# youtalk/opencv-ar

Hardware: AMD Instinct MI355X
Metric: frames/sec at 1920x1080, 16 markers/frame; 1/2/4/8 MI355X (higher is better)
Workload: dtype u8

## Files before the change

include/ocvar_hip.h:

```cpp
#ifndef OCVAR_HIP_H
#define OCVAR_HIP_H

#include <stddef.h>
#include <stdint.h>

#ifdef __cplusplus
extern "C" {
#endif

typedef struct { int width, height; double cameraMatrix[9]; double distCoeffs[5]; double glProjection[16]; } OcvarCamera;
typedef struct { int width, height; double scale; long long code[4]; } OcvarTemplate;
typedef struct {
    double glMatrix[16]; int templateId; int markerId; double score; float square[8]; double aspectRatio;
} OcvarMarker;

typedef struct {
    int markerId, templateId, orient, valid;
    long long bit;
    float square[8];
    float patPoint[8];
} OcvarCandidate;

typedef struct OcvarHip OcvarHip;

enum {
    OCVAR_OK = 0,
    OCVAR_E_NO_DEVICE = -1,
    OCVAR_E_ARG = -2,
    OCVAR_E_HIP = -3,
    OCVAR_E_CAPACITY = -4
};

enum { OCVAR_MAX_TEMPLATES = 4096, OCVAR_MAX_TEMPLATE_SIZES = 16, OCVAR_MAX_QUADS = 256, OCVAR_MAX_MARKERS = 64,
       OCVAR_MAX_QUADS_EX = 1792 ,
       OCVAR_MAX_QUADS_DENSE = 16384, OCVAR_MAX_MARKERS_DENSE = 4096  };

int ocvar_hip_create(OcvarHip** ctx, int device, int max_width, int max_height, int max_batch);
int ocvar_hip_create_ex(OcvarHip** ctx, int device, int max_width, int max_height, int max_batch, int max_quads);
int ocvar_hip_create_dense(OcvarHip** ctx, int device, int max_width, int max_height, int max_batch, int max_quads, int max_markers);
int ocvar_hip_max_markers(const OcvarHip* ctx);
void ocvar_hip_destroy(OcvarHip* ctx);
const char* ocvar_hip_last_error(const OcvarHip* ctx);
int ocvar_hip_capacity_flags(const OcvarHip* ctx);

typedef struct OcvarGate OcvarGate;
int ocvar_hip_gate_create(OcvarGate** gate, int device, int width);
int ocvar_hip_gate_create_lanes(OcvarGate** gate, int device, int width, int lanes);
int ocvar_hip_gate_lanes(const OcvarGate* gate);
void ocvar_hip_gate_destroy(OcvarGate* gate);
int ocvar_hip_set_gate(OcvarHip* ctx, OcvarGate* gate);

int ocvar_hip_set_templates(OcvarHip* ctx, const OcvarTemplate* templates, int n);
int ocvar_hip_set_camera(OcvarHip* ctx, const OcvarCamera* camera);

enum { OCVAR_FMT_BGR = 0, OCVAR_FMT_RGB = 1, OCVAR_FMT_BGRA = 2, OCVAR_FMT_RGBA = 3, OCVAR_FMT_GRAY = 4 };
int ocvar_hip_set_input_format(OcvarHip* ctx, int format);

enum { OCVAR_MAX_REFINE_HALF_WIN = 15 };
int ocvar_hip_set_corner_refine(OcvarHip* ctx, int half_win, int max_iter, float eps);

enum { OCVAR_MAX_BOARD_MARKERS = 256 };
typedef struct { int templateId; int pad; double corner[8]; } OcvarBoardMarker;
typedef struct {
    double glMatrix[16];
    double rvec[3], tvec[3];
    double rms;
    int n_markers;
    int status;
} OcvarBoardPose;
int ocvar_hip_set_board(OcvarHip* ctx, const OcvarBoardMarker* markers, int n);
int ocvar_hip_board_poses(OcvarHip* ctx, OcvarBoardPose* poses, int n_frames);
int ocvar_hip_board_poses_to_device(OcvarHip* ctx, OcvarBoardPose* d_poses, void* stream);

enum { OCVAR_MAX_OVERLAYS = 64, OCVAR_MAX_OVERLAY_SIDE = 1024 };
int ocvar_hip_set_overlay(OcvarHip* ctx, int template_id, const uint8_t* h_rgba, int width, int height, int row_stride);
int ocvar_hip_render(OcvarHip* ctx, uint8_t* d_frames, int width, int height, int row_stride, size_t frame_stride, int format,
                     void* stream);
int ocvar_hip_render_records(OcvarHip* ctx, uint8_t* d_frames, int width, int height, int row_stride, size_t frame_stride,
                             int n_frames, int format, const OcvarMarker* d_markers, const int* d_counts, int records_per_frame,
                             void* stream);

enum { OCVAR_MAX_PATCH_SIDE = 256, OCVAR_PATCH_FLIP_ROWS = 1, OCVAR_PATCH_MATCHED_ONLY = 2 };
int ocvar_hip_patches(OcvarHip* ctx, const uint8_t* d_frames, int width, int height, int row_stride, size_t frame_stride, int format,
                      uint8_t* d_patches, int patch_w, int patch_h, int records_per_frame, int flags, int* d_status, void* stream);
int ocvar_hip_patches_records(OcvarHip* ctx, const uint8_t* d_frames, int width, int height, int row_stride, size_t frame_stride,
                              int n_frames, int format, const OcvarMarker* d_markers, const int* d_counts, int records_per_frame,
                              uint8_t* d_patches, int patch_w, int patch_h, int flags, int* d_status, void* stream);

int ocvar_hip_detect_device(OcvarHip* ctx, uint8_t* d_bgr, int width, int height, int row_stride, size_t frame_stride,
                            int n_frames, int grey_in_place, const OcvarMarker* prev, const int* prev_counts,
                            OcvarMarker* markers, int* counts, int max_per_frame);
int ocvar_hip_enqueue(OcvarHip* ctx, uint8_t* d_bgr, int width, int height, int row_stride, size_t frame_stride,
                      int n_frames, int grey_in_place, const OcvarMarker* prev, const int* prev_counts, void* stream);
int ocvar_hip_collect(OcvarHip* ctx, OcvarMarker* markers, int* counts, int max_per_frame);
int ocvar_hip_enqueue_tracked(OcvarHip* ctx, uint8_t* d_bgr, int width, int height, int row_stride, size_t frame_stride,
                              int n_frames, int grey_in_place, const OcvarMarker* d_prev, const int* d_prev_counts, void* stream);
int ocvar_hip_ready(OcvarHip* ctx);
int ocvar_hip_set_result_limit(OcvarHip* ctx, int max_per_frame);

enum { OCVAR_TUNE_CROP_PHASES = 1,
       OCVAR_TUNE_MID_STEPS = 2,
       OCVAR_TUNE_MID_BLOCKS = 3, OCVAR_TUNE_LONG_BLOCKS = 4, OCVAR_TUNE_SHORT_BLOCKS = 5,
       OCVAR_TUNE_MIN_UNITS = 6,
       OCVAR_TUNE_GATE_MODE = 8,
       OCVAR_TUNE_HP_MASK = 7 };
int ocvar_hip_set_tuning(OcvarHip* ctx, int knob, int value);
const char* ocvar_hip_build_info(void);

void* ocvar_hip_stream(const OcvarHip* ctx);

int ocvar_hip_results_to_device(OcvarHip* ctx, OcvarMarker* d_markers, int* d_counts, void* stream);
int ocvar_hip_results_to_device_ex(OcvarHip* ctx, OcvarMarker* d_markers, int* d_counts, int max_per_frame, void* stream);

typedef struct OcvarPipe OcvarPipe;
int ocvar_hip_pipe_create(OcvarPipe** pipe, int device, int max_width, int max_height, int chunk_frames, int n_contexts, int gate_width);
void ocvar_hip_pipe_destroy(OcvarPipe* pipe);
const char* ocvar_hip_pipe_last_error(const OcvarPipe* pipe);
int ocvar_hip_pipe_set_templates(OcvarPipe* pipe, const OcvarTemplate* templates, int n);
int ocvar_hip_pipe_set_camera(OcvarPipe* pipe, const OcvarCamera* camera);
int ocvar_hip_pipe_detect_device(OcvarPipe* pipe, uint8_t* d_bgr, int width, int height, int row_stride, size_t frame_stride,
                                 long long n_frames, int grey_in_place, OcvarMarker* markers, int* counts, int max_per_frame);
int ocvar_hip_pipe_track_device(OcvarPipe* pipe, uint8_t* d_bgr, int width, int height, int row_stride, size_t frame_stride,
                                long long n_streams, int grey_in_place, int reset, OcvarMarker* markers, int* counts, int max_per_frame);

enum { OCVAR_E_BUSY = -6 };
int ocvar_hip_pipe_submit(OcvarPipe* pipe, uint8_t* d_bgr, int width, int height, int row_stride, size_t frame_stride, int n_frames,
                          int grey_in_place, long long tag);
int ocvar_hip_pipe_collect(OcvarPipe* pipe, long long* tag, OcvarMarker* markers, int* counts, int max_per_frame);
int ocvar_hip_pipe_in_flight(const OcvarPipe* pipe);
int ocvar_hip_pipe_set_result_limit(OcvarPipe* pipe, int max_per_frame);
int ocvar_hip_pipe_set_input_format(OcvarPipe* pipe, int format);
// ... 26 lines not shown
```

opencv-ar_amd/__init__.py:

```python
import ctypes as C
import os

import numpy as np

_HERE = os.path.dirname(os.path.abspath(__file__))
LIB_DIR = os.path.join(_HERE, "lib")
HIP_LIB = os.environ.get("OCVAR_HIP_LIB") or os.path.join(LIB_DIR, "libocvar_hip.so")
SYNTH_LIB = os.path.join(LIB_DIR, "libocvar_synth.so")
HOST_LIB = os.path.join(LIB_DIR, "libopencv-ar.so.1.0.0")

MAX_TEMPLATES, MAX_TEMPLATE_SIZES, MAX_QUADS, MAX_MARKERS = 4096, 16, 256, 64
MAX_QUADS_EX, MAX_QUADS_DENSE, MAX_MARKERS_DENSE = 1792, 16384, 4096

HIP_SYMBOLS = [
    "ocvar_hip_create", "ocvar_hip_create_ex", "ocvar_hip_create_dense", "ocvar_hip_max_markers", "ocvar_hip_capacity_flags", "ocvar_hip_gate_create", "ocvar_hip_gate_create_lanes", "ocvar_hip_gate_lanes", "ocvar_hip_gate_destroy", "ocvar_hip_set_gate", "ocvar_hip_ready", "ocvar_hip_set_result_limit",
    "ocvar_hip_pipe_create", "ocvar_hip_pipe_destroy", "ocvar_hip_pipe_last_error", "ocvar_hip_pipe_set_templates", "ocvar_hip_pipe_set_camera",
    "ocvar_hip_pipe_detect_device", "ocvar_hip_pipe_track_device", "ocvar_hip_pipe_submit", "ocvar_hip_pipe_collect", "ocvar_hip_pipe_in_flight", "ocvar_hip_pipe_set_result_limit", "ocvar_hip_set_input_format", "ocvar_hip_pipe_set_input_format", "ocvar_hip_set_corner_refine", "ocvar_hip_pipe_set_corner_refine", "ocvar_hip_enqueue_tracked", "ocvar_hip_build_info", "ocvar_hip_set_tuning", "ocvar_hip_destroy", "ocvar_hip_last_error", "ocvar_hip_set_templates", "ocvar_hip_set_camera",
    "ocvar_hip_detect_device", "ocvar_hip_enqueue", "ocvar_hip_collect", "ocvar_hip_detect_host", "ocvar_hip_find_squares",
    "ocvar_hip_debug_gray", "ocvar_hip_debug_binary", "ocvar_hip_debug_masks", "ocvar_hip_debug_frame_quads", "ocvar_hip_debug_candidates",
    "ocvar_hip_stage_ms", "ocvar_hip_stream", "ocvar_hip_stage_stamps", "ocvar_hip_counters", "ocvar_hip_results_to_device", "ocvar_hip_results_to_device_ex", "ocvar_hip_debug_calibrate",
    "ocvar_hip_set_board", "ocvar_hip_board_poses", "ocvar_hip_board_poses_to_device",
    "ocvar_hip_set_overlay", "ocvar_hip_render", "ocvar_hip_render_records",
    "ocvar_hip_patches", "ocvar_hip_patches_records",
]
INPUT_FORMATS = {"bgr": 0, "rgb": 1, "bgra": 2, "rgba": 3, "gray": 4}
FORMAT_BPP = {0: 3, 1: 3, 2: 4, 3: 4, 4: 1}


def input_format_code(fmt):
    if isinstance(fmt, str) and fmt.lower() in INPUT_FORMATS:
        return INPUT_FORMATS[fmt.lower()]
    if isinstance(fmt, int) and not isinstance(fmt, bool) and fmt in FORMAT_BPP:
        return fmt
    raise ValueError(f"unknown input format {fmt!r}: one of {sorted(INPUT_FORMATS)}")


def frame_shape_bpp(shape, fmt):
    bpp = FORMAT_BPP[input_format_code(fmt)]
    if bpp == 1:
        if len(shape) != 3:
            raise ValueError(f"gray frames are [n, H, W], got {tuple(shape)}")
    elif len(shape) != 4 or shape[3] != bpp:
        raise ValueError(f"frames in this format are [n, H, W, {bpp}], got {tuple(shape)}")
    return shape[0], shape[1], shape[2]


MAX_REFINE_HALF_WIN = 15


def corner_refine_args(half_win, max_iter, eps):
    for name, v in (("half_win", half_win), ("max_iter", max_iter)):
        if isinstance(v, bool) or not isinstance(v, (int, np.integer)):
            raise ValueError(f"{name} must be an int, got {v!r}")
    if not 0 <= half_win <= MAX_REFINE_HALF_WIN:
        raise ValueError(f"half_win must be 0 .. {MAX_REFINE_HALF_WIN}, got {half_win}")
    if not 1 <= max_iter <= 100:
        raise ValueError(f"max_iter must be 1 .. 100, got {max_iter}")
    if isinstance(eps, bool) or not isinstance(eps, (int, float, np.integer, np.floating)) or not 0 <= float(eps) < 1e30:
        raise ValueError(f"eps must be a number >= 0, got {eps!r}")
    return int(half_win), int(max_iter), float(eps)


MAX_BOARD_MARKERS = 256
MAX_OVERLAYS, MAX_OVERLAY_SIDE = 64, 1024
MAX_PATCH_SIDE, PATCH_FLIP_ROWS, PATCH_MATCHED_ONLY = 256, 1, 2


class BoardMarker(C.Structure):
    _fields_ = [("templateId", C.c_int), ("pad", C.c_int), ("corner", C.c_double * 8)]


BOARD_DTYPE = np.dtype([("glMatrix", "<f8", (16,)), ("rvec", "<f8", (3,)), ("tvec", "<f8", (3,)), ("rms", "<f8"),
                        ("n_markers", "<i4"), ("status", "<i4")], align=True)
assert C.sizeof(BoardMarker) == 72 and BOARD_DTYPE.itemsize == 192


def grid_board(template_ids, cols, rows, length, separation):
    if len(template_ids) > cols * rows:
        raise ValueError(f"{len(template_ids)} templates for a {cols} x {rows} grid")
    out = []
    for k, t in enumerate(template_ids):
        x0, y0 = (k % cols) * (length + separation), (k // cols) * (length + separation)
        out.append((int(t), np.array([[x0, y0], [x0 + length, y0], [x0 + length, y0 + length], [x0, y0 + length]], np.float64)))
    return out


STAGE_NAMES = ["binarise_frames", "follow1_frames", "follow2_frames", "follow3_frames", "order_crops", "binarise_crops",
               "follow1_crops", "follow2_crops", "follow3_crops", "decode", "dedupe_pose", "batch_total"]


class Camera(C.Structure):
    _fields_ = [("width", C.c_int), ("height", C.c_int), ("cameraMatrix", C.c_double * 9),
                ("distCoeffs", C.c_double * 5), ("glProjection", C.c_double * 16)]


class Template(C.Structure):
    _fields_ = [("width", C.c_int), ("height", C.c_int), ("scale", C.c_double), ("code", C.c_longlong * 4)]


class Marker(C.Structure):
    _fields_ = [("glMatrix", C.c_double * 16), ("templateId", C.c_int), ("markerId", C.c_int),
                ("score", C.c_double), ("square", C.c_float * 8), ("aspectRatio", C.c_double)]


class Candidate(C.Structure):
    _fields_ = [("markerId", C.c_int), ("templateId", C.c_int), ("orient", C.c_int), ("valid", C.c_int),
                ("bit", C.c_longlong), ("square", C.c_float * 8), ("patPoint", C.c_float * 8)]


MARKER_DTYPE = np.dtype([("glMatrix", "<f8", (16,)), ("templateId", "<i4"), ("markerId", "<i4"), ("score", "<f8"),
                         ("square", "<f4", (8,)), ("aspectRatio", "<f8")], align=True)
assert C.sizeof(Camera) == 248 and C.sizeof(Template) == 48 and C.sizeof(Marker) == 184 and MARKER_DTYPE.itemsize == 184


class OcvarError(RuntimeError):
    pass


_hip = None


def hip_lib():
    global _hip
    if _hip is None:
        if not os.path.exists(HIP_LIB):
            raise OcvarError(f"{HIP_LIB} is missing: run `python -c 'import __graft_entry__ as g; g.build()'` "
                             "(there is no CPU fallback for the detection path)")
        try:
            import torch
        except ImportError:
            pass
        lib = C.CDLL(HIP_LIB)
        vp, i, sz = C.c_void_p, C.c_int, C.c_size_t
        lib.ocvar_hip_create.argtypes = [C.POINTER(vp), i, i, i, i]
        lib.ocvar_hip_create_dense.argtypes = [C.POINTER(vp), i, i, i, i, i, i]
        lib.ocvar_hip_max_markers.argtypes = [vp]
        lib.ocvar_hip_destroy.argtypes = [vp]
        lib.ocvar_hip_gate_create.argtypes = [C.POINTER(vp), i, i]
        lib.ocvar_hip_gate_create_lanes.argtypes = [C.POINTER(vp), i, i, i]
        lib.ocvar_hip_gate_lanes.argtypes = [vp]
        lib.ocvar_hip_gate_destroy.argtypes = [vp]
        lib.ocvar_hip_gate_destroy.restype = None
        lib.ocvar_hip_set_gate.argtypes = [vp, vp]
        lib.ocvar_hip_ready.argtypes = [vp]
        lib.ocvar_hip_set_result_limit.argtypes = [vp, i]
        lib.ocvar_hip_pipe_create.argtypes = [C.POINTER(vp), i, i, i, i, i, i]
        lib.ocvar_hip_pipe_destroy.argtypes = [vp]
        lib.ocvar_hip_pipe_destroy.restype = None
        lib.ocvar_hip_pipe_last_error.argtypes = [vp]
        lib.ocvar_hip_pipe_last_error.restype = C.c_char_p
        lib.ocvar_hip_pipe_set_templates.argtypes = [vp, vp, i]
        lib.ocvar_hip_pipe_set_camera.argtypes = [vp, vp]
        lib.ocvar_hip_pipe_detect_device.argtypes = [vp, vp, i, i, i, sz, C.c_longlong, i, vp, vp, i]
        lib.ocvar_hip_pipe_track_device.argtypes = [vp, vp, i, i, i, sz, C.c_longlong, i, i, vp, vp, i]
        lib.ocvar_hip_pipe_submit.argtypes = [vp, vp, i, i, i, sz, i, i, C.c_longlong]
        lib.ocvar_hip_pipe_collect.argtypes = [vp, C.POINTER(C.c_longlong), vp, vp, i]
        lib.ocvar_hip_pipe_in_flight.argtypes = [vp]
        lib.ocvar_hip_pipe_set_result_limit.argtypes = [vp, i]
        lib.ocvar_hip_pipe_set_input_format.argtypes = [vp, i]
        lib.ocvar_hip_set_input_format.argtypes = [vp, i]
        lib.ocvar_hip_set_corner_refine.argtypes = [vp, i, i, C.c_float]
        lib.ocvar_hip_pipe_set_corner_refine.argtypes = [vp, i, i, C.c_float]
        lib.ocvar_hip_enqueue_tracked.argtypes = [vp, vp, i, i, i, sz, i, i, vp, vp, vp]
        lib.ocvar_hip_set_tuning.argtypes = [vp, i, i]
        lib.ocvar_hip_build_info.argtypes = []
        lib.ocvar_hip_build_info.restype = C.c_char_p
        lib.ocvar_hip_destroy.restype = None
        lib.ocvar_hip_last_error.argtypes = [vp]
        lib.ocvar_hip_last_error.restype = C.c_char_p
        lib.ocvar_hip_set_templates.argtypes = [vp, vp, i]
        lib.ocvar_hip_set_camera.argtypes = [vp, vp]
        lib.ocvar_hip_detect_device.argtypes = [vp, vp, i, i, i, sz, i, i, vp, vp, vp, vp, i]
        lib.ocvar_hip_enqueue.argtypes = [vp, vp, i, i, i, sz, i, i, vp, vp, vp]
        lib.ocvar_hip_collect.argtypes = [vp, vp, vp, i]
        lib.ocvar_hip_detect_host.argtypes = [vp, vp, i, i, i, sz, i, i, vp, vp, vp, vp, i]
        lib.ocvar_hip_find_squares.argtypes = [vp, vp, i, i, i, vp, i, vp]
        lib.ocvar_hip_debug_gray.argtypes = [vp, i, vp]
        lib.ocvar_hip_debug_binary.argtypes = [vp, i, vp]
        lib.ocvar_hip_debug_masks.argtypes = [vp, i, vp]
        lib.ocvar_hip_debug_frame_quads.argtypes = [vp, i, vp, vp]
        lib.ocvar_hip_debug_candidates.argtypes = [vp, i, vp, i, vp]
        lib.ocvar_hip_stage_ms.argtypes = [vp, vp, i]
        lib.ocvar_hip_counters.argtypes = [vp, vp, i]
        lib.ocvar_hip_stage_stamps.argtypes = [vp, vp, vp, i]
        lib.ocvar_hip_stream.argtypes = [vp]
        lib.ocvar_hip_stream.restype = vp
        lib.ocvar_hip_results_to_device.argtypes = [vp, vp, vp, vp]
        lib.ocvar_hip_results_to_device_ex.argtypes = [vp, vp, vp, i, vp]
        lib.ocvar_hip_debug_calibrate.argtypes = [vp, sz]
        lib.ocvar_hip_set_board.argtypes = [vp, vp, i]
        lib.ocvar_hip_board_poses.argtypes = [vp, vp, i]
        lib.ocvar_hip_board_poses_to_device.argtypes = [vp, vp, vp]
        lib.ocvar_hip_set_overlay.argtypes = [vp, i, vp, i, i, i]
        lib.ocvar_hip_render.argtypes = [vp, vp, i, i, i, sz, i, vp]
        lib.ocvar_hip_render_records.argtypes = [vp, vp, i, i, i, sz, i, i, vp, vp, i, vp]
        lib.ocvar_hip_patches.argtypes = [vp, vp, i, i, i, sz, i, vp, i, i, i, i, vp, vp]
        lib.ocvar_hip_patches_records.argtypes = [vp, vp, i, i, i, sz, i, i, vp, vp, i, vp, i, i, i, vp, vp]
        _hip = lib
    return _hip


_host = None


def host_lib():
    global _host
    if _host is None:
        if not os.path.exists(HOST_LIB):
            raise OcvarError(f"{HOST_LIB} is missing: run `python -c 'import __graft_entry__ as g; g.build()'`")
        hip_lib()
        lib = C.CDLL(HOST_LIB)
        lib.cvarLoadTemplateTag.argtypes = [C.c_void_p, C.c_char_p, C.c_double]
        lib.cvarReadCamera.argtypes = [C.c_char_p, C.c_void_p]
        lib.cvarCameraScale.argtypes = [C.c_void_p, C.c_int, C.c_int]
        _host = lib
    return _host


TEMPLATE_DIR = os.path.join(os.path.dirname(_HERE), "assets", "templates")


def load_templates(paths, scale=0.01):
    out = []
    for path in paths:
        t = Template()
        if host_lib().cvarLoadTemplateTag(C.byref(t), os.fsencode(path), scale) != 1:
            raise OcvarError(f"cvarLoadTemplateTag failed for {path}")
        out.append(t)
    return out


def default_camera(width, height, filename=None):
    cam = Camera()
    if host_lib().cvarReadCamera(os.fsencode(filename) if filename else None, C.byref(cam)) != 1:
        raise OcvarError(f"cvarReadCamera failed for {filename}")
    host_lib().cvarCameraScale(C.byref(cam), width, height)
    return cam


def _ptr(a):
    return C.c_void_p(a.ctypes.data) if a is not None else None


class Gate:

    def __init__(self, width=2, device=0, lanes=0):
        self._lib = hip_lib()
        self._g = C.c_void_p()
        rc = self._lib.ocvar_hip_gate_create_lanes(C.byref(self._g), device, width, lanes)
        if rc != 0:
            raise OcvarError(f"ocvar_hip_gate_create_lanes failed ({rc})")

    @property
    def lanes(self):
        return self._lib.ocvar_hip_gate_lanes(self._g)

    def __del__(self):
        if getattr(self, "_g", None):
            self._lib.ocvar_hip_gate_destroy(self._g)
            self._g = None


class Pipe:

    input_format = INPUT_FORMATS["bgr"]

    def __init__(self, max_width, max_height, chunk_frames=2048, n_contexts=4, gate_width=2, device=0):
        self._lib = hip_lib()
        self._p = C.c_void_p()
        self.chunk_frames = chunk_frames
        rc = self._lib.ocvar_hip_pipe_create(C.byref(self._p), device, max_width, max_height, chunk_frames, n_contexts, gate_width)
        if rc != 0:
            msg = self._lib.ocvar_hip_pipe_last_error(self._p).decode() if self._p else ""
            self.close()
            raise OcvarError(f"ocvar_hip_pipe_create failed ({rc}): {msg}")

    def close(self):
        if getattr(self, "_p", None):
            self._lib.ocvar_hip_pipe_destroy(self._p)
            self._p = None

    def __del__(self):
        try:
            self.close()
        except Exception:
            pass

    def _check(self, rc, what):
        if rc != 0:
            raise OcvarError(f"{what} failed ({rc}): {self._lib.ocvar_hip_pipe_last_error(self._p).decode()}")

    def set_templates(self, templates):
        arr = (Template * len(templates))(*templates)
        self._check(self._lib.ocvar_hip_pipe_set_templates(self._p, arr, len(templates)), "pipe_set_templates")

    def set_camera(self, camera):
        self._check(self._lib.ocvar_hip_pipe_set_camera(self._p, C.byref(camera)), "pipe_set_camera")

    def set_input_format(self, fmt):
        code = input_format_code(fmt)
        self._check(self._lib.ocvar_hip_pipe_set_input_format(self._p, code), "pipe_set_input_format")
        self.input_format = code

    def set_corner_refine(self, half_win=5, max_iter=30, eps=0.1):
        w, it, e = corner_refine_args(half_win, max_iter, eps)
        self._check(self._lib.ocvar_hip_pipe_set_corner_refine(self._p, w, it, e), "pipe_set_corner_refine")

    def detect_device(self, d_ptr, width, height, n_frames, row_stride=None, frame_stride=None, grey_in_place=False, max_per_frame=MAX_MARKERS):
        row_stride = row_stride or FORMAT_BPP[self.input_format] * width
        frame_stride = frame_stride or row_stride * height
        markers = np.zeros((n_frames, max_per_frame), MARKER_DTYPE)
        counts = np.zeros(n_frames, np.int32)
        self._check(self._lib.ocvar_hip_pipe_detect_device(self._p, d_ptr, width, height, row_stride, frame_stride, n_frames,
                                                           int(grey_in_place), _ptr(markers), _ptr(counts), max_per_frame), "pipe_detect_device")
        return markers, counts

    def submit(self, d_ptr, width, height, n_frames, tag=0, row_stride=None, frame_stride=None, grey_in_place=False):
        row_stride = row_stride or FORMAT_BPP[self.input_format] * width
        frame_stride = frame_stride or row_stride * height
        rc = self._lib.ocvar_hip_pipe_submit(self._p, d_ptr, width, height, row_stride, frame_stride, n_frames, int(grey_in_place), tag)
        if rc == -6:
            return False
        self._check(rc, "pipe_submit")
        return True

    def collect(self, max_frames, max_per_frame=MAX_MARKERS):
        rows = max(max_frames, self.chunk_frames)
        markers = np.zeros((rows, max_per_frame), MARKER_DTYPE)
        counts = np.zeros(rows, np.int32)
        tag = C.c_longlong(0)
        n = self._lib.ocvar_hip_pipe_collect(self._p, C.byref(tag), _ptr(markers), _ptr(counts), max_per_frame)
        if n < 0:
            self._check(n, "pipe_collect")
        if n == 0:
            return None
        return tag.value, markers[:n], counts[:n]

    def in_flight(self):
# ... 284 lines not shown
```

opencv-ar_amd/csrc/api.hip:

```cpp
#include "kernels.h"
#include "lanes_core.h"
#include <algorithm>
#include <cstdio>
#include <cstdlib>
#include <cstring>
#include <mutex>
#include <new>
#include <string>
#include <thread>
#include <vector>

using namespace ocvar;

static_assert(sizeof(TemplateRec) == sizeof(OcvarTemplate) && sizeof(TemplateRec) == 48, "CvarTemplate layout");
static_assert(MAX_SIZE_CLASSES == OCVAR_MAX_TEMPLATE_SIZES, "size classes");
static_assert(sizeof(CameraRec) == sizeof(OcvarCamera) && sizeof(CameraRec) == 248, "CvarCamera layout");
static_assert(sizeof(MarkerRec) == sizeof(OcvarMarker) && sizeof(MarkerRec) == 184, "CvarMarker layout");
static_assert(sizeof(BoardEntry) == sizeof(OcvarBoardMarker) && sizeof(BoardEntry) == 72, "OcvarBoardMarker layout");
static_assert(sizeof(BoardPose) == sizeof(OcvarBoardPose) && sizeof(BoardPose) == 192, "OcvarBoardPose layout");

struct OcvarGate {
    int device = 0;
    std::mutex mu;
    LaneSched sched;
// ... 166 lines not shown
    if ((rc = dev_alloc(c, &w.ring_frame, B))) return rc;
    if ((rc = dev_alloc(c, &w.ring_crop, (size_t)w.cap_crop_rois))) return rc;
    if ((rc = dev_alloc(c, &w.sq_recs, B * max_quads))) return rc;
    if ((rc = dev_alloc(c, &w.prev, B * M))) return rc;
    if ((rc = dev_alloc(c, &w.n_prev, B))) return rc;
    if ((rc = dev_alloc(c, &w.reserve, B * M))) return rc;
    if ((rc = dev_alloc(c, &w.n_reserve, B))) return rc;
    if ((rc = dev_alloc(c, &w.markers, B * M))) return rc;
    if ((rc = dev_alloc(c, &w.pose_jobs, B * M))) return rc;
    if (dense) {
        const int nc = track_grid_cells(max_width, max_height, &w.track_gw, &w.track_gh);
        w.decode_slices = std::max(4, std::min(64, max_quads / 64));
        for (w.order_chunk = 2; w.order_chunk < max_quads && w.order_chunk < ORDER_CHUNK;) w.order_chunk <<= 1;
        if ((rc = dev_alloc(c, &w.sorted_starts, B * max_quads))) return rc;
        if ((rc = dev_alloc(c, &w.sq_tmp, B * max_quads * 8))) return rc;
        if ((rc = dev_alloc(c, &w.trk_cells, B * (nc + 1)))) return rc;
        if ((rc = dev_alloc(c, &w.trk_fill, B * nc))) return rc;
        if ((rc = dev_alloc(c, &w.trk_items, B * 4 * max_quads))) return rc;
        if ((rc = dev_alloc(c, &w.trk_next, B * (max_quads + 1)))) return rc;
        if ((rc = dev_alloc(c, &w.surv, B * max_quads))) return rc;
        if ((rc = dev_alloc(c, &w.src, B * M))) return rc;
    }
    if ((rc = dev_alloc(c, &w.n_markers, B))) return rc;
    if ((rc = dev_alloc(c, &w.templates, (size_t)MAXT))) return rc;
    if ((rc = dev_alloc(c, &w.sizes, (size_t)MAX_SIZE_CLASSES))) return rc;
    if ((rc = dev_alloc(c, &w.lut, (size_t)4 * MAXT))) return rc;
    if ((rc = dev_alloc(c, &w.group_off, (size_t)MAXT + 1))) return rc;
    if ((rc = dev_alloc(c, &w.group_members, (size_t)MAXT))) return rc;
    if ((rc = dev_alloc(c, &w.camera, (size_t)1))) return rc;
    if ((rc = dev_alloc(c, &w.counters, (size_t)CNT_COUNT))) return rc;

    w.crop_pixels = reinterpret_cast<unsigned long long*>(w.counters + CNT_CROP_PIXELS);
    HIP_TRY(c, hipMemset(w.n_prev, 0, B * sizeof(int)));
    HIP_TRY(c, hipMemset(w.counters, 0, CNT_COUNT * sizeof(int)));
    HIP_TRY(c, hipHostMalloc((void**)&c->h_markers, B * M * sizeof(MarkerRec)));
    HIP_TRY(c, hipHostMalloc((void**)&c->h_counts, B * sizeof(int)));
    HIP_TRY(c, hipHostMalloc((void**)&c->h_prev, B * M * sizeof(MarkerRec)));
    HIP_TRY(c, hipHostMalloc((void**)&c->h_prev_counts, B * sizeof(int)));
    HIP_TRY(c, hipHostMalloc((void**)&c->h_counters, CNT_COUNT * sizeof(int)));
    return OCVAR_OK;
}

static void gate_detach(OcvarHip* c);

extern "C" void ocvar_hip_destroy(OcvarHip* c) {
    if (!c) return;
    (void)hipSetDevice(c->device);
    gate_detach(c);
    if (c->stream) (void)hipStreamSynchronize(c->stream);
    for (void* p : c->allocs) (void)hipFree(p);
    if (c->ws.sq_codes) (void)hipFree(c->ws.sq_codes);
    if (c->ws.sq_match) (void)hipFree(c->ws.sq_match);
    if (c->d_frames) (void)hipFree(c->d_frames);
    for (auto p : c->h_stage)
        if (p) (void)hipHostFree(p);
    for (auto p : c->h_grey)
        if (p) (void)hipHostFree(p);
    if (c->h_markers) (void)hipHostFree(c->h_markers);
    if (c->h_counts) (void)hipHostFree(c->h_counts);
    if (c->h_prev) (void)hipHostFree(c->h_prev);
    if (c->h_prev_counts) (void)hipHostFree(c->h_prev_counts);
    if (c->h_counters) (void)hipHostFree(c->h_counters);
    if (c->h_board_poses) (void)hipHostFree(c->h_board_poses);
    if (c->h_overlays) {
        if (c->ovl_used) (void)hipEventSynchronize(c->ovl_done);
        for (auto& t : c->h_overlays->tex)
            if (t.px) (void)hipFree(const_cast<uint32_t*>(t.px));
        delete c->h_overlays;
    }
    if (c->ovl_done) (void)hipEventDestroy(c->ovl_done);
    for (auto& e : c->ev)
        if (e) (void)hipEventDestroy(e);
    for (auto& e : c->h2d_done) (void)hipEventDestroy(e);
    if (c->computed) (void)hipEventDestroy(c->computed);
    if (c->ordered) (void)hipEventDestroy(c->ordered);
    if (c->copied) (void)hipEventDestroy(c->copied);
    if (c->h2d_stream) (void)hipStreamDestroy(c->h2d_stream);
    if (c->d2h_stream) (void)hipStreamDestroy(c->d2h_stream);
    if (c->hp_stream) (void)hipStreamDestroy(c->hp_stream);
    if (c->stream) (void)hipStreamDestroy(c->stream);
    delete c;
}

static int lanes_of_this_process(int forced) {
    return lanes_for_queues(parse_queue_count(std::getenv("GPU_MAX_HW_QUEUES")), forced);
}

extern "C" int ocvar_hip_gate_create(OcvarGate** out, int device, int width) { return ocvar_hip_gate_create_lanes(out, device, width, 0); }

extern "C" int ocvar_hip_gate_create_lanes(OcvarGate** out, int device, int width, int lanes) {
    if (!out || width < 1 || width > 64 || lanes < 0 || lanes > LANES_MAX) return OCVAR_E_ARG;
    *out = nullptr;
    if (hipSetDevice(device) != hipSuccess) return OCVAR_E_NO_DEVICE;
    OcvarGate* g = new (std::nothrow) OcvarGate();
    if (!g) return OCVAR_E_HIP;
    g->device = device;
    lane_sched_init(&g->sched, lanes_of_this_process(lanes), width);
    g->ring.resize(256);
    bool ok = true;
    g->lanes.assign((size_t)g->sched.n_lanes, nullptr);
    for (auto& l : g->lanes) ok = ok && hipStreamCreateWithFlags(&l, hipStreamNonBlocking) == hipSuccess;
    for (auto& e : g->ring) ok = ok && hipEventCreateWithFlags(&e, hipEventDisableTiming) == hipSuccess;
    if (!ok) {
        ocvar_hip_gate_destroy(g);
        return OCVAR_E_HIP;
    }
    *out = g;
    return OCVAR_OK;
}

extern "C" int ocvar_hip_gate_lanes(const OcvarGate* g) { return g ? g->sched.n_lanes : OCVAR_E_ARG; }

static void lane_release(OcvarHip* c) {
    OcvarGate* g = c->gate;
    if (!g) return;
    std::lock_guard<std::mutex> lock(g->mu);
    if (c->lane >= 0) lane_retire(&g->sched, c->lane);
    c->lane = -1;
}

static hipError_t batch_wait(OcvarHip* c) {
    if (!c->on_lane) return hipStreamSynchronize(c->last_stream);
    return hipEventSynchronize(c->copy_pending ? c->copied : c->ev[12]);
}

static void gate_detach(OcvarHip* c) {
    OcvarGate* g = c->gate;
    if (!g) return;
    if (c->pending && c->on_lane) {
        (void)batch_wait(c);
        c->on_lane = false;
        c->copy_pending = false;
        c->last_stream = c->stream;
    }
    lane_release(c);
    {
        std::lock_guard<std::mutex> lock(g->mu);
        auto& a = g->attached;
        a.erase(std::remove(a.begin(), a.end(), c), a.end());
    }
    c->gate = nullptr;
}

extern "C" void ocvar_hip_gate_destroy(OcvarGate* g) {
    if (!g) return;
    (void)hipSetDevice(g->device);
    for (auto& l : g->lanes)
        if (l) (void)hipStreamSynchronize(l);
    while (!g->attached.empty()) gate_detach(g->attached.back());
    for (auto& l : g->lanes)
        if (l) (void)hipStreamDestroy(l);
    for (auto& e : g->ring)
        if (e) (void)hipEventDestroy(e);
    delete g;
}

extern "C" int ocvar_hip_set_gate(OcvarHip* c, OcvarGate* g) {
    if (!c || (g && g->device != c->device)) return OCVAR_E_ARG;
    if (g == c->gate) return OCVAR_OK;
    (void)hipSetDevice(c->device);
    gate_detach(c);
    c->gate = g;
    if (g) {
        std::lock_guard<std::mutex> lock(g->mu);
        g->attached.push_back(c);
    }
    return OCVAR_OK;
}

static int lane_batch_done(void* user, int i) {
    OcvarHip* o = (*static_cast<std::vector<OcvarHip*>*>(user))[(size_t)i];
    if (hipEventQuery(o->ev[12]) == hipSuccess) return 1;
    (void)hipGetLastError();
    return 0;
}
static int gate_place(OcvarGate* g) {
    std::lock_guard<std::mutex> lock(g->mu);
    int* lane_of[64];
    const int n = (int)std::min<size_t>(g->attached.size(), 64);
    for (int i = 0; i < n; i++) lane_of[i] = &g->attached[(size_t)i]->lane;
    return lane_place(&g->sched, lane_of, n, lane_batch_done, &g->attached);
}

static hipError_t gate_enter(OcvarGate* g, hipStream_t s) {
    if (!g) return hipSuccess;
    const long long wait_for = gate_wait_for(&g->sched);
    if (wait_for < 0) return hipSuccess;
    return hipStreamWaitEvent(s, g->ring[(size_t)wait_for % g->ring.size()], 0);
}
static hipError_t gate_leave(OcvarGate* g, hipStream_t s) {
    if (!g) return hipSuccess;
    const hipError_t e = hipEventRecord(g->ring[(size_t)g->sched.issued % g->ring.size()], s);
    (void)gate_ticket(&g->sched);
    return e;
// ... 1082 lines not shown
```

opencv-ar_amd/csrc/kernels.h:

```cpp
#pragma once
#include "hd.h"
#include "decode_core.h"
#include "pose_core.h"
#include "tail_core.h"
#include "refine_core.h"
#include "board_core.h"
#include "overlay_core.h"
#include "patch_core.h"
#include "ocvar_hip.h"

namespace ocvar {

constexpr int MAXQ_DEFAULT = OCVAR_MAX_QUADS;
constexpr int MAXM = OCVAR_MAX_MARKERS;
constexpr int MAXT = OCVAR_MAX_TEMPLATES;
constexpr int MARCH_HALO_L = 2, MARCH_HALO_R = 2;
constexpr int MARCH_STRIP = 4 * (64 - MARCH_HALO_L - MARCH_HALO_R);
static_assert(MARCH_STRIP == GRAY_PANEL_COLS && 4 * MARCH_HALO_L == GRAY_PANEL_LEAD && 4 * 64 == GRAY_PANEL_BYTES, "a grey panel is what one wave of the frame kernel converts");
constexpr int MARCH_CROP_ROWS = 252;
constexpr int MARCH_STAGE = 512;
constexpr int BACK_STEPS = 32;
constexpr int PRE_STEPS = 8;
constexpr int SHORT_STEPS = 96;
constexpr int MID_STEPS = 1536;
// ... 65 lines not shown
    int* crop_of;
    Roi* rois_crop;
    TileDesc* tiles_crop;
    unsigned long long* crop_pixels;
    QuadRec* quads_crop;
    unsigned long long* best_crop;
    int* ring_frame;
    int* ring_crop;
    int* crop_min_rest;
    SquareRec* sq_recs;
    long long* sq_codes;
    int* sq_match;
    MarkerRec* prev;
    int* n_prev;
    int* reserve;
    int* n_reserve;
    int* pose_jobs;
    MarkerRec* markers;
    int* sorted_starts;
    float* sq_tmp;
    int* trk_cells;
    int* trk_fill;
    int* trk_items;
    int* trk_next;
    int* surv;
    int* src;
    int* n_markers;
    TemplateRec* templates;
    SizeClass* sizes;
    LutEntry* lut;
    int* group_off;
    int* group_members;
    CameraRec* camera;
    int* counters;
};

int input_format_bpp(int format);

void launch_binarise_frames(const Workspace& ws, const uint8_t* d_bgr, int row_stride, size_t frame_stride, int grey_in_place,
                            int format, hipStream_t stream);
void launch_binarise_crops(const Workspace& ws, hipStream_t stream);
void launch_ring_quads_frames(const Workspace& ws, hipStream_t stream);
void launch_ring_quads_crops(const Workspace& ws, hipStream_t stream);
void launch_follow_frames(const Workspace& ws, hipStream_t stream);
void launch_follow_crops(const Workspace& ws, hipStream_t stream);
void launch_follow_mid_frames(const Workspace& ws, hipStream_t stream);
void launch_follow_mid_crops(const Workspace& ws, hipStream_t stream);
void launch_follow_long_frames(const Workspace& ws, hipStream_t stream);
void launch_follow_long_crops(const Workspace& ws, hipStream_t stream);
void launch_order_and_crops(const Workspace& ws, hipStream_t stream);
void launch_decode(const Workspace& ws, hipStream_t stream);
void launch_finalise(const Workspace& ws, const RefineArgs& refine, hipStream_t stream);
void launch_refine_corners(const Workspace& ws, const RefineArgs& refine, hipStream_t stream);

struct BoardArgs {
    int n;
    const BoardEntry* entries;
    const int* map;
    BoardPose* poses;
};
void launch_board_poses(const Workspace& ws, const BoardArgs& board, hipStream_t stream);

struct OverlayArgs {
    const OverlayTable* table;
    OverlayDraw* draws;
    OverlayBox* boxes;
};
void launch_overlay(const OverlayArgs& oa, uint8_t* frames, int W, int H, long long row_stride, long long frame_stride, int n_frames,
                    int format, const MarkerRec* recs, const int* counts, int stride, hipStream_t stream);

struct PatchArgs {
    const uint8_t* frames;
    int W, H;
    long long row_stride, frame_stride;
    const MarkerRec* recs;
    const int* counts;
    int rec_stride;
    uint8_t* patches;
    int pw, ph, slots, flags;
    int* status;
};
void launch_patches(const PatchArgs& a, int n_frames, int format, hipStream_t stream);

}
```

opencv-ar_amd/csrc/lanes_core.h:

```cpp
#pragma once

namespace ocvar {

constexpr int LANES_MAX = 8;
constexpr int HW_QUEUES_DEFAULT = 4;

inline int lanes_for_queues(int hw_queues, int forced) {
    int n = forced > 0 ? forced : (hw_queues > 0 ? hw_queues : HW_QUEUES_DEFAULT);
    return n < 1 ? 1 : (n > LANES_MAX ? LANES_MAX : n);
}

inline int parse_queue_count(const char* text) {
    if (!text) return 0;
    long v = 0;
    for (const char* p = text; *p; p++) {
        if (*p < '0' || *p > '9') return 0;
        v = v * 10 + (*p - '0');
        if (v > 1 << 20) return 0;
    }
    return (int)v;
}

struct LaneSched {
    int n_lanes = 1;
    int width = 1;
    int outstanding[LANES_MAX] = {};
    unsigned long long newest[LANES_MAX] = {};
    unsigned long long placed = 0;
    unsigned long long issued = 0;
};

inline void lane_sched_init(LaneSched* s, int n_lanes, int width) {
    *s = LaneSched();
    s->n_lanes = n_lanes < 1 ? 1 : (n_lanes > LANES_MAX ? LANES_MAX : n_lanes);
    s->width = width < 1 ? 1 : width;
}

inline int lane_choose(const LaneSched* s) {
    int best = 0;
    for (int l = 1; l < s->n_lanes; l++)
        if (s->outstanding[l] < s->outstanding[best] ||
            (s->outstanding[l] == s->outstanding[best] && s->newest[l] < s->newest[best]))
            best = l;
    return best;
}

inline void lane_book(LaneSched* s, int lane) {
    s->outstanding[lane]++;
    s->newest[lane] = ++s->placed;
}

inline void lane_retire(LaneSched* s, int lane) {
    if (lane >= 0 && lane < s->n_lanes && s->outstanding[lane] > 0) s->outstanding[lane]--;
}

typedef int (*LaneDoneFn)(void* user, int batch);
inline void lane_refresh(LaneSched* s, int* const* lane_of, int n, LaneDoneFn done, void* user) {
    for (int i = 0; i < n; i++)
        if (*lane_of[i] >= 0 && done(user, i)) {
            lane_retire(s, *lane_of[i]);
            *lane_of[i] = -1;
        }
}

inline int lane_place(LaneSched* s, int* const* lane_of, int n, LaneDoneFn done, void* user) {
    lane_refresh(s, lane_of, n, done, user);
    const int lane = lane_choose(s);
    lane_book(s, lane);
    return lane;
}

inline long long gate_wait_for(const LaneSched* s) {
    const long long w = (long long)s->issued - s->width;
    return w < 0 ? -1 : w;
}
inline long long gate_ticket(LaneSched* s) { return (long long)s->issued++; }

}
```

Baseline: 251,300.

## Probe stream-to-hardware-queue grouping and spread gate lanes across distinct queues

At gate creation the code now makes extra candidate streams and runs a timing probe: a long sleep kernel on one stream plus timestamp kernels on the others reveals which streams share a hardware queue. Lanes are then picked from distinct queue groups, and the scheduler balances load per group rather than per stream. The goal is to stop two lanes from serialising on the same hardware queue when work is spread across lanes. The cost is extra startup work (probe kernels, synchronisation, creating and destroying streams) and a dependence on timing heuristics that may misclassify streams.

```diff
diff --git a/include/ocvar_hip.h b/include/ocvar_hip.h
--- a/include/ocvar_hip.h
+++ b/include/ocvar_hip.h
@@ -46,7 +46,11 @@
 typedef struct OcvarGate OcvarGate;
 int ocvar_hip_gate_create(OcvarGate** gate, int device, int width);
 int ocvar_hip_gate_create_lanes(OcvarGate** gate, int device, int width, int lanes);
+enum { OCVAR_GATE_NO_PROBE = 1 };
+int ocvar_hip_gate_create_ex(OcvarGate** gate, int device, int width, int lanes, int flags);
 int ocvar_hip_gate_lanes(const OcvarGate* gate);
+int ocvar_hip_gate_lane_group(const OcvarGate* gate, int lane);
+void* ocvar_hip_gate_lane_stream(const OcvarGate* gate, int lane);
 void ocvar_hip_gate_destroy(OcvarGate* gate);
 int ocvar_hip_set_gate(OcvarHip* ctx, OcvarGate* gate);
 
diff --git a/opencv-ar_amd/__init__.py b/opencv-ar_amd/__init__.py
--- a/opencv-ar_amd/__init__.py
+++ b/opencv-ar_amd/__init__.py
@@ -13,7 +13,7 @@
 MAX_QUADS_EX, MAX_QUADS_DENSE, MAX_MARKERS_DENSE = 1792, 16384, 4096
 
 HIP_SYMBOLS = [
-    "ocvar_hip_create", "ocvar_hip_create_ex", "ocvar_hip_create_dense", "ocvar_hip_max_markers", "ocvar_hip_capacity_flags", "ocvar_hip_gate_create", "ocvar_hip_gate_create_lanes", "ocvar_hip_gate_lanes", "ocvar_hip_gate_destroy", "ocvar_hip_set_gate", "ocvar_hip_ready", "ocvar_hip_set_result_limit",
+    "ocvar_hip_create", "ocvar_hip_create_ex", "ocvar_hip_create_dense", "ocvar_hip_max_markers", "ocvar_hip_capacity_flags", "ocvar_hip_gate_create", "ocvar_hip_gate_create_lanes", "ocvar_hip_gate_create_ex", "ocvar_hip_gate_lanes", "ocvar_hip_gate_lane_group", "ocvar_hip_gate_lane_stream", "ocvar_hip_gate_destroy", "ocvar_hip_set_gate", "ocvar_hip_ready", "ocvar_hip_set_result_limit",
     "ocvar_hip_pipe_create", "ocvar_hip_pipe_destroy", "ocvar_hip_pipe_last_error", "ocvar_hip_pipe_set_templates", "ocvar_hip_pipe_set_camera",
     "ocvar_hip_pipe_detect_device", "ocvar_hip_pipe_track_device", "ocvar_hip_pipe_submit", "ocvar_hip_pipe_collect", "ocvar_hip_pipe_in_flight", "ocvar_hip_pipe_set_result_limit", "ocvar_hip_set_input_format", "ocvar_hip_pipe_set_input_format", "ocvar_hip_set_corner_refine", "ocvar_hip_pipe_set_corner_refine", "ocvar_hip_enqueue_tracked", "ocvar_hip_build_info", "ocvar_hip_set_tuning", "ocvar_hip_destroy", "ocvar_hip_last_error", "ocvar_hip_set_templates", "ocvar_hip_set_camera",
     "ocvar_hip_detect_device", "ocvar_hip_enqueue", "ocvar_hip_collect", "ocvar_hip_detect_host", "ocvar_hip_find_squares",
@@ -138,7 +138,11 @@
         lib.ocvar_hip_destroy.argtypes = [vp]
         lib.ocvar_hip_gate_create.argtypes = [C.POINTER(vp), i, i]
         lib.ocvar_hip_gate_create_lanes.argtypes = [C.POINTER(vp), i, i, i]
+        lib.ocvar_hip_gate_create_ex.argtypes = [C.POINTER(vp), i, i, i, i]
         lib.ocvar_hip_gate_lanes.argtypes = [vp]
+        lib.ocvar_hip_gate_lane_group.argtypes = [vp, i]
+        lib.ocvar_hip_gate_lane_stream.argtypes = [vp, i]
+        lib.ocvar_hip_gate_lane_stream.restype = vp
         lib.ocvar_hip_gate_destroy.argtypes = [vp]
         lib.ocvar_hip_gate_destroy.restype = None
         lib.ocvar_hip_set_gate.argtypes = [vp, vp]
@@ -244,16 +248,27 @@
 
 class Gate:
 
-    def __init__(self, width=2, device=0, lanes=0):
+    NO_PROBE = 1
+
+    def __init__(self, width=2, device=0, lanes=0, probe=True):
         self._lib = hip_lib()
         self._g = C.c_void_p()
-        rc = self._lib.ocvar_hip_gate_create_lanes(C.byref(self._g), device, width, lanes)
+        rc = self._lib.ocvar_hip_gate_create_ex(C.byref(self._g), device, width, lanes, 0 if probe else self.NO_PROBE)
         if rc != 0:
-            raise OcvarError(f"ocvar_hip_gate_create_lanes failed ({rc})")
+            raise OcvarError(f"ocvar_hip_gate_create_ex failed ({rc})")
 
     @property
     def lanes(self):
         return self._lib.ocvar_hip_gate_lanes(self._g)
+
+    @property
+    def lane_groups(self):
+        return [self._lib.ocvar_hip_gate_lane_group(self._g, l) for l in range(self.lanes)]
+
+    def lane_stream(self, lane):
+        if not 0 <= lane < self.lanes:
+            raise IndexError(f"lane {lane} of {self.lanes}")
+        return self._lib.ocvar_hip_gate_lane_stream(self._g, lane)
 
     def __del__(self):
         if getattr(self, "_g", None):
diff --git a/opencv-ar_amd/csrc/api.hip b/opencv-ar_amd/csrc/api.hip
--- a/opencv-ar_amd/csrc/api.hip
+++ b/opencv-ar_amd/csrc/api.hip
@@ -272,24 +272,37 @@
     delete c;
 }
 
-static int lanes_of_this_process(int forced) {
-    return lanes_for_queues(parse_queue_count(std::getenv("GPU_MAX_HW_QUEUES")), forced);
-}
-
-extern "C" int ocvar_hip_gate_create(OcvarGate** out, int device, int width) { return ocvar_hip_gate_create_lanes(out, device, width, 0); }
+extern "C" int ocvar_hip_gate_create(OcvarGate** out, int device, int width) { return ocvar_hip_gate_create_ex(out, device, width, 0, 0); }
 
 extern "C" int ocvar_hip_gate_create_lanes(OcvarGate** out, int device, int width, int lanes) {
-    if (!out || width < 1 || width > 64 || lanes < 0 || lanes > LANES_MAX) return OCVAR_E_ARG;
+    return ocvar_hip_gate_create_ex(out, device, width, lanes, 0);
+}
+
+extern "C" int ocvar_hip_gate_create_ex(OcvarGate** out, int device, int width, int lanes, int flags) {
+    if (!out || width < 1 || width > 64 || lanes < 0 || lanes > LANES_MAX || (flags & ~OCVAR_GATE_NO_PROBE)) return OCVAR_E_ARG;
     *out = nullptr;
     if (hipSetDevice(device) != hipSuccess) return OCVAR_E_NO_DEVICE;
     OcvarGate* g = new (std::nothrow) OcvarGate();
     if (!g) return OCVAR_E_HIP;
     g->device = device;
-    lane_sched_init(&g->sched, lanes_of_this_process(lanes), width);
+    const int hw_queues = parse_queue_count(std::getenv("GPU_MAX_HW_QUEUES"));
+    lane_sched_init(&g->sched, lanes_for_queues(hw_queues, lanes), width);
+    const int n_lanes = g->sched.n_lanes;
     g->ring.resize(256);
     bool ok = true;
-    g->lanes.assign((size_t)g->sched.n_lanes, nullptr);
-    for (auto& l : g->lanes) ok = ok && hipStreamCreateWithFlags(&l, hipStreamNonBlocking) == hipSuccess;
+    const bool probe = !(flags & OCVAR_GATE_NO_PROBE);
+    const int n_cand = probe ? probe_candidates(hw_queues, n_lanes) : n_lanes;
+    hipStream_t cand[CANDIDATES_MAX] = {};
+    int group[CANDIDATES_MAX], chosen[LANES_MAX], lane_group[LANES_MAX];
+    for (int i = 0; i < n_cand; i++) ok = ok && hipStreamCreateWithFlags(&cand[i], hipStreamNonBlocking) == hipSuccess;
+    for (int i = 0; i < n_cand; i++) group[i] = -1;
+    if (ok && probe) ok = probe_stream_groups(cand, n_cand, group) == hipSuccess;
+    lane_select(group, n_cand, n_lanes, chosen, lane_group);
+    lane_sched_set_groups(&g->sched, lane_group);
+    g->lanes.assign((size_t)n_lanes, nullptr);
+    for (int l = 0; l < n_lanes; l++) std::swap(g->lanes[(size_t)l], cand[chosen[l]]);
+    for (int i = 0; i < n_cand; i++)
+        if (cand[i]) (void)hipStreamDestroy(cand[i]);
     for (auto& e : g->ring) ok = ok && hipEventCreateWithFlags(&e, hipEventDisableTiming) == hipSuccess;
     if (!ok) {
         ocvar_hip_gate_destroy(g);
@@ -300,6 +313,12 @@
 }
 
 extern "C" int ocvar_hip_gate_lanes(const OcvarGate* g) { return g ? g->sched.n_lanes : OCVAR_E_ARG; }
+extern "C" int ocvar_hip_gate_lane_group(const OcvarGate* g, int lane) {
+    return g && lane >= 0 && lane < g->sched.n_lanes ? g->sched.group[lane] : OCVAR_E_ARG;
+}
+extern "C" void* ocvar_hip_gate_lane_stream(const OcvarGate* g, int lane) {
+    return g && lane >= 0 && lane < g->sched.n_lanes ? (void*)g->lanes[(size_t)lane] : nullptr;
+}
 
 static void lane_release(OcvarHip* c) {
     OcvarGate* g = c->gate;
diff --git a/opencv-ar_amd/csrc/kernels.h b/opencv-ar_amd/csrc/kernels.h
--- a/opencv-ar_amd/csrc/kernels.h
+++ b/opencv-ar_amd/csrc/kernels.h
@@ -171,4 +171,6 @@
 };
 void launch_patches(const PatchArgs& a, int n_frames, int format, hipStream_t stream);
 
+hipError_t probe_stream_groups(const hipStream_t* cand, int n, int* group);
+
 }
diff --git a/opencv-ar_amd/csrc/lane_probe.hip b/opencv-ar_amd/csrc/lane_probe.hip
--- /dev/null
+++ b/opencv-ar_amd/csrc/lane_probe.hip
@@ -0,0 +1,84 @@
+#include "kernels.h"
+#include "lanes_core.h"
+#include <chrono>
+
+namespace ocvar_probe {
+
+__global__ void lane_probe_wait_kernel(unsigned long long* out, unsigned long long ticks, int max_iter) {
+    if (threadIdx.x != 0) return;
+    const unsigned long long t0 = wall_clock64();
+    unsigned long long t = t0;
+    for (int i = 0; i < max_iter && t - t0 < ticks; i++) {
+        __builtin_amdgcn_s_sleep(32);
+        t = wall_clock64();
+    }
+    out[0] = t0;
+    out[1] = t;
+}
+
+__global__ void lane_probe_stamp_kernel(unsigned long long* out) {
+    if (threadIdx.x == 0) *out = wall_clock64();
+}
+
+}
+
+namespace ocvar {
+using ocvar_probe::lane_probe_stamp_kernel;
+using ocvar_probe::lane_probe_wait_kernel;
+
+static hipError_t sync_all(const hipStream_t* cand, int n) {
+    hipError_t first = hipSuccess;
+    for (int i = 0; i < n; i++) {
+        const hipError_t e = hipStreamSynchronize(cand[i]);
+        if (first == hipSuccess) first = e;
+    }
+    return first;
+}
+
+hipError_t probe_stream_groups(const hipStream_t* cand, int n, int* group) {
+    for (int i = 0; i < n; i++) group[i] = -1;
+    if (n < 1 || n > CANDIDATES_MAX) return hipErrorInvalidValue;
+    unsigned long long* h = nullptr;
+    hipError_t e = hipHostMalloc((void**)&h, (2 + CANDIDATES_MAX) * sizeof(unsigned long long));
+    if (e != hipSuccess) return e;
+    lane_probe_wait_kernel<<<1, 64, 0, cand[0]>>>(h, 0, 1);
+    for (int i = 0; i < n; i++) lane_probe_stamp_kernel<<<1, 64, 0, cand[i]>>>(h + 2 + i);
+    e = hipGetLastError();
+    const hipError_t es = sync_all(cand, n);
+    if (e == hipSuccess) e = es;
+
+    bool gave_up = false;
+    for (int gid = 0; e == hipSuccess && !gave_up; gid++) {
+        int ref = -1, open = 0;
+        for (int i = n - 1; i >= 0; i--)
+            if (group[i] < 0) ref = i, open++;
+        if (ref < 0) break;
+        if (open == 1) {
+            group[ref] = gid;
+            break;
+        }
+        bool filed = false;
+        for (int attempt = 0; attempt < 2 && e == hipSuccess && !filed; attempt++) {
+            const unsigned long long wait_ticks = PROBE_WAIT_TICKS << attempt;
+            for (int i = 0; i < 2 + CANDIDATES_MAX; i++) h[i] = 0;
+            const auto t0 = std::chrono::steady_clock::now();
+            lane_probe_wait_kernel<<<1, 64, 0, cand[ref]>>>(h, wait_ticks, (int)(wait_ticks / 100 * 16));
+            for (int i = 0; i < n; i++)
+                if (i != ref && group[i] < 0) lane_probe_stamp_kernel<<<1, 64, 0, cand[i]>>>(h + 2 + i);
+            const double filled_us = std::chrono::duration<double, std::micro>(std::chrono::steady_clock::now() - t0).count();
+            e = hipGetLastError();
+            const hipError_t es2 = sync_all(cand, n);
+            if (e == hipSuccess) e = es2;
+            if (e != hipSuccess) break;
+            if (filled_us * 100.0 > (double)wait_ticks * 0.5) continue;
+            filed = probe_round_file(group, n, ref, gid, h + 2, h[0], h[1], wait_ticks);
+        }
+        if (!filed) gave_up = true;
+    }
+    if (gave_up || e != hipSuccess)
+        for (int i = 0; i < n; i++) group[i] = -1;
+    (void)hipHostFree(h);
+    return e;
+}
+
+}
diff --git a/opencv-ar_amd/csrc/lanes_core.h b/opencv-ar_amd/csrc/lanes_core.h
--- a/opencv-ar_amd/csrc/lanes_core.h
+++ b/opencv-ar_amd/csrc/lanes_core.h
@@ -21,9 +21,68 @@
     return (int)v;
 }
 
+constexpr int CANDIDATES_MAX = 16;
+
+inline int probe_candidates(int hw_queues, int n_lanes) {
+    const long long q = hw_queues > 0 ? hw_queues : HW_QUEUES_DEFAULT;
+    long long c = 2 * q + 2;
+    if (c > CANDIDATES_MAX) c = CANDIDATES_MAX;
+    if (c < n_lanes) c = n_lanes;
+    return (int)c;
+}
+
+constexpr unsigned long long PROBE_WAIT_TICKS = 30000;
+constexpr unsigned long long PROBE_GUARD_TICKS = 2000;
+constexpr unsigned long long PROBE_LATE_TICKS = 10000;
+enum { PROBE_DISTINCT = 0, PROBE_SHARED = 1, PROBE_AMBIGUOUS = 2 };
+inline int probe_classify(unsigned long long stamp, unsigned long long ref_end) {
+    if (stamp + PROBE_GUARD_TICKS <= ref_end) return PROBE_DISTINCT;
+    if (stamp >= ref_end && stamp - ref_end <= PROBE_LATE_TICKS) return PROBE_SHARED;
+    return PROBE_AMBIGUOUS;
+}
+
+inline bool probe_round_file(int* group, int n, int ref, int gid, const unsigned long long* stamp, unsigned long long ref_start,
+                             unsigned long long ref_end, unsigned long long wait_ticks) {
+    if (ref_end < ref_start || ref_end - ref_start < wait_ticks) return false;
+    for (int i = 0; i < n; i++)
+        if (i != ref && group[i] < 0 && probe_classify(stamp[i], ref_end) == PROBE_AMBIGUOUS) return false;
+    for (int i = 0; i < n; i++)
+        if (i != ref && group[i] < 0 && probe_classify(stamp[i], ref_end) == PROBE_SHARED) group[i] = gid;
+    group[ref] = gid;
+    return true;
+}
+
+inline int lane_select(const int* group, int n_cand, int n_lanes, int* chosen, int* lane_group) {
+    if (n_cand > CANDIDATES_MAX) n_cand = CANDIDATES_MAX;
+    if (n_lanes > n_cand) n_lanes = n_cand;
+    bool probed = n_cand > 0;
+    for (int i = 0; i < n_cand; i++) probed = probed && group[i] >= 0;
+    if (!probed) {
+        for (int l = 0; l < n_lanes; l++) chosen[l] = l, lane_group[l] = -1;
+        return n_lanes;
+    }
+    bool used[CANDIDATES_MAX] = {};
+    int groups[CANDIDATES_MAX], n_groups = 0, n = 0;
+    for (int i = 0; i < n_cand; i++) {
+        bool seen = false;
+        for (int k = 0; k < n_groups; k++) seen = seen || groups[k] == group[i];
+        if (seen) continue;
+        groups[n_groups++] = group[i];
+        if (n < n_lanes) used[i] = true, chosen[n] = i, lane_group[n] = group[i], n++;
+    }
+    for (int k = 0; n < n_lanes; k = (k + 1) % n_groups)
+        for (int i = 0; i < n_cand; i++)
+            if (!used[i] && group[i] == groups[k]) {
+                used[i] = true, chosen[n] = i, lane_group[n] = group[i], n++;
+                break;
+            }
+    return n_lanes;
+}
+
 struct LaneSched {
     int n_lanes = 1;
     int width = 1;
+    int group[LANES_MAX] = {-1, -1, -1, -1, -1, -1, -1, -1};
     int outstanding[LANES_MAX] = {};
     unsigned long long newest[LANES_MAX] = {};
     unsigned long long placed = 0;
@@ -36,12 +95,27 @@
     s->width = width < 1 ? 1 : width;
 }
 
+inline void lane_sched_set_groups(LaneSched* s, const int* lane_group) {
+    for (int l = 0; l < s->n_lanes; l++) s->group[l] = lane_group[l];
+}
+
+inline int lane_group_load(const LaneSched* s, int lane) {
+    if (s->group[lane] < 0) return s->outstanding[lane];
+    int sum = 0;
+    for (int l = 0; l < s->n_lanes; l++)
+        if (s->group[l] == s->group[lane]) sum += s->outstanding[l];
+    return sum;
+}
+
 inline int lane_choose(const LaneSched* s) {
-    int best = 0;
-    for (int l = 1; l < s->n_lanes; l++)
-        if (s->outstanding[l] < s->outstanding[best] ||
-            (s->outstanding[l] == s->outstanding[best] && s->newest[l] < s->newest[best]))
-            best = l;
+    int best = 0, best_load = lane_group_load(s, 0);
+    for (int l = 1; l < s->n_lanes; l++) {
+        const int load = lane_group_load(s, l);
+        if (load < best_load ||
+            (load == best_load && (s->outstanding[l] < s->outstanding[best] ||
+                                   (s->outstanding[l] == s->outstanding[best] && s->newest[l] < s->newest[best]))))
+            best = l, best_load = load;
+    }
     return best;
 }
 
```

After: 251,700, median of 2. About the same (+0.2%).
